# LogicTronixInc/Event-Camera-Clustering-and-Optical-Flow-Estimation

Hardware: AMD Instinct MI355X
Metric: Mevents/s (downsample+cluster+corner) (higher is better)
Workload: dtype u16xy/i64t (int), fp32 k-means; 1 GPU; e2e hash-downsample(8192-event windows) -> k-means k=16 (10 iters) on reps -> SAE+FAST arc corners (16384-event slices) -> 15x15 NMS; 346x260 sensor; 20004864 events/GPU/step (BASELINE configs C2-C4); events_per_gpu=20004864, events_total=20004864, preset=c4, reps_per_gpu=7697279, width=346, height=260, k=16, kmeans_iters=10, parallelism=time-window shards x1, launch=eager launches, streams=two streams sharing all CUs

## Files before the change

### event-camera-clustering-and-optical-flow-estimation_amd/csrc/corner_flags.hip

```cpp
#include "corner_common.hpp"

namespace {

#ifndef ECC_FLAG_THREADS
#define ECC_FLAG_THREADS 256
#endif
constexpr int kFlagThreads = ECC_FLAG_THREADS;
#ifndef ECC_FLAG_QUADS
#define ECC_FLAG_QUADS 8
#endif
constexpr int kFlagQuads = ECC_FLAG_QUADS;
constexpr int kFlagBatch = kFlagQuads * kFlagThreads;

template <bool kStaged>
__device__ __forceinline__ uint32_t corner_bit(uint32_t v, const CornerGeom &g, const uint32_t *sb,
                                               const uint32_t *__restrict__ rg, int j) {
    const int x = ecc::xy_x(v), y = ecc::xy_y(v);
    if (x >= g.W || y >= g.H) return 0u;
    const int tile = (y / kTile) * g.tiles_x + x / kTile;
    const int lp = (y % kTile) * kTile + x % kTile;
    if (kStaged) return (sb[tile * kSegWords + (lp >> 5)] >> (lp & 31)) & 1u;
    return (rg[(int64_t)tile * kSegWords + (lp >> 5)] >> (lp & 31)) & 1u;
}

template <bool kStaged, bool kCand>
__global__ void __launch_bounds__(kFlagThreads)
flags_event_kernel(const uint32_t *__restrict__ xy, CornerGeom g, const uint32_t *__restrict__ res,
                   const int32_t *__restrict__ first_border, uint8_t *__restrict__ flags, uint32_t *__restrict__ cand,
                   int32_t *__restrict__ n_cand) {
    extern __shared__ uint32_t sb[];
    __shared__ int ctot[kFlagQuads][kFlagThreads / 64];
    const int64_t s = blockIdx.x;
    const int64_t lo = s * g.S;
    const int len = (int)((lo + g.S < g.n ? lo + g.S : g.n) - lo);
    const int j = (int)(s % kGroup);
    const int live_end = s < g.first_detect ? 0 : (g.border_mode == 1 ? min(len, max(first_border[s], 0)) : len);
    const uint32_t *rg = res + s * g.seg_stride;
    const bool vec = ((lo + (int64_t)(reinterpret_cast<uintptr_t>(flags) & 3)) & 3) == 0;
    const int n4 = vec ? len / 4 : 0;
    const int lane = threadIdx.x & 63, wave = threadIdx.x >> 6;
    const __amdgpu_buffer_rsrc_t vq = ecc::buffer_view(xy + lo, (uint32_t)n4 * 16u);
    uint4 pre[kFlagQuads];
    auto load_batch = [&](int q0) {
#pragma unroll
        for (int u = 0; u < kFlagQuads; ++u)
            pre[u] = ecc::buffer_load_u128(vq, threadIdx.x * 16u, (uint32_t)(q0 + u * kFlagThreads) * 16u);
        __builtin_amdgcn_sched_barrier(0);
    };
    load_batch(0);
    if (kStaged && live_end > 0) {
        const int total = g.n_tiles * kSegWords;
        const __amdgpu_buffer_rsrc_t vr = ecc::buffer_view(rg, (uint32_t)total * 4u);
        for (int k0 = 0; k0 < total; k0 += 16 * kFlagThreads) {
            uint4 a[4];
#pragma unroll
            for (int b = 0; b < 4; ++b) a[b] = ecc::buffer_load_u128(vr, (uint32_t)(k0 + 4 * (b * kFlagThreads + (int)threadIdx.x)) * 4u);
            __builtin_amdgcn_sched_barrier(0);
#pragma unroll
            for (int b = 0; b < 4; ++b) {
                const int k = k0 + 4 * (b * kFlagThreads + (int)threadIdx.x);
                if (k + 3 < total) {
                    *reinterpret_cast<uint4 *>(sb + k) = a[b];
                } else {
                    if (k < total) sb[k] = a[b].x;
                    if (k + 1 < total) sb[k + 1] = a[b].y;
                    if (k + 2 < total) sb[k + 2] = a[b].z;
                }
            }
        }
    }
    __syncthreads();
    auto quad_flags = [&](int i, const uint4 v) {
        return corner_bit<kStaged>(v.x, g, sb, rg, j) | (i + 1 < live_end ? corner_bit<kStaged>(v.y, g, sb, rg, j) << 8 : 0u) |
               (i + 2 < live_end ? corner_bit<kStaged>(v.z, g, sb, rg, j) << 16 : 0u) |
               (i + 3 < live_end ? corner_bit<kStaged>(v.w, g, sb, rg, j) << 24 : 0u);
    };
    const uint64_t lt = lane == 0 ? 0ull : (~0ull >> (64 - lane));
    int base = 0;
    uint32_t *dst = cand + lo;
    for (int q0 = 0; q0 < n4; q0 += kFlagBatch) {
        if (q0 > 0) load_batch(q0);
        uint32_t f[kFlagQuads];
        int pfx[kFlagQuads];
#pragma unroll
        for (int u = 0; u < kFlagQuads; ++u) {
            const int q = q0 + u * kFlagThreads + (int)threadIdx.x;
            const int i = 4 * q;
            f[u] = (q < n4 && i < live_end) ? quad_flags(i, pre[u]) : 0u;
            if (q < n4) *reinterpret_cast<uint32_t *>(flags + lo + i) = f[u];
            if constexpr (kCand) {
                const int c = __popc(f[u]);
                const uint64_t b0 = __ballot(c & 1), b1 = __ballot(c & 2), b2 = __ballot(c & 4);
                pfx[u] = __popcll(b0 & lt) + 2 * __popcll(b1 & lt) + 4 * __popcll(b2 & lt);
                if (lane == 0) ctot[u][wave] = __popcll(b0) + 2 * __popcll(b1) + 4 * __popcll(b2);
            }
        }
        if constexpr (kCand) {
            __syncthreads();
#pragma unroll
            for (int u = 0; u < kFlagQuads; ++u) {
                int off = base + pfx[u];
#pragma unroll
                for (int w = 0; w < kFlagThreads / 64; ++w) {
                    const int tw = ctot[u][w];
                    off += w < wave ? tw : 0;
                    base += tw;
                }
                if (f[u]) {
                    if (f[u] & 0x1u) dst[off++] = pre[u].x;
                    if (f[u] & 0x100u) dst[off++] = pre[u].y;
                    if (f[u] & 0x10000u) dst[off++] = pre[u].z;
                    if (f[u] & 0x1000000u) dst[off++] = pre[u].w;
                }
            }
            __syncthreads();
        }
    }
    if constexpr (kCand) {
        if (threadIdx.x == 0) {
            for (int i = 4 * n4; i < len; ++i) {
                const uint32_t v = xy[lo + i];
                const uint32_t fb = i < live_end ? corner_bit<kStaged>(v, g, sb, rg, j) : 0u;
                flags[lo + i] = (uint8_t)fb;
                if (fb) dst[base++] = v;
            }
            n_cand[s] = base;
        }
    } else {
        for (int i = 4 * n4 + threadIdx.x; i < len; i += kFlagThreads)
            flags[lo + i] = (uint8_t)(i < live_end ? corner_bit<kStaged>(xy[lo + i], g, sb, rg, j) : 0u);
    }
}

}

int ecc::corner::launch_flags(ecc_ctx *ctx, hipStream_t s, const uint32_t *xy, const CornerGeom &g, const GroupImages &gi,
                              const int32_t *first_border, uint8_t *corner_flags, uint32_t *cand, int32_t *n_cand) {
    ECC_TIMED(ctx, s, "flags_kernel");
    constexpr size_t kLdsMax = kFlagDynLdsMax;
    const size_t lds = (size_t)g.n_tiles * kSegWords * sizeof(uint32_t);
    if (lds <= kLdsMax) {
        const auto fn = cand ? &flags_event_kernel<true, true> : &flags_event_kernel<true, false>;
        if (lds > 65536)
            if (int rc = ecc::allow_dynamic_lds(ctx, fn, (int)kLdsMax, "flags LDS")) return rc;
        if (cand)
            hipLaunchKernelGGL((flags_event_kernel<true, true>), dim3((unsigned)g.n_slices), dim3(kFlagThreads), lds, s,
                               xy, g, (const uint32_t *)gi.res, first_border, corner_flags, cand, n_cand);
        else
            hipLaunchKernelGGL((flags_event_kernel<true, false>), dim3((unsigned)g.n_slices), dim3(kFlagThreads), lds,
                               s, xy, g, (const uint32_t *)gi.res, first_border, corner_flags, nullptr, nullptr);
    } else {
        if (cand) return ECC_ERR_INVALID;
        hipLaunchKernelGGL((flags_event_kernel<false, false>), dim3((unsigned)g.n_slices), dim3(kFlagThreads), 0, s,
                           xy, g, (const uint32_t *)gi.res, first_border, corner_flags, nullptr, nullptr);
    }
    return ECC_OK;
}
```

### event-camera-clustering-and-optical-flow-estimation_amd/csrc/downsample.hip

```cpp
#include "ecc_internal.hpp"

namespace {

constexpr int kThreads = 512;
constexpr int kMaxWindow = 16384;
constexpr int kBuckets = 8192;
constexpr uint32_t kEmpty = 0x7fffffffu;
constexpr uint32_t kRepeatBit = 0x80000000u;

template <bool kQuads>
__device__ inline void load4(const uint32_t *__restrict__ xy, int64_t g, int64_t n, uint32_t (&v)[4]) {
    if constexpr (kQuads) {
        const int64_t n4 = n >> 2, qi = g >> 2;
        const uint4 q = reinterpret_cast<const uint4 *>(xy)[qi < n4 ? qi : n4 - 1];
        v[0] = q.x; v[1] = q.y; v[2] = q.z; v[3] = q.w;
    } else {
#pragma unroll
        for (int k = 0; k < 4; ++k) v[k] = xy[g + k < n ? g + k : n - 1];
    }
}

template <int NT, int MAXC, bool kQuads>
__global__ void __launch_bounds__(NT)
downsample_hash_kernel(const uint32_t *__restrict__ xy, int64_t n, int window, int n_chunks,
                       int x_max, int y_max, int mult_x, int mult_y,
                       uint32_t *__restrict__ rep_xy, uint32_t *__restrict__ rep_idx,
                       int32_t *__restrict__ win_unique, int32_t *__restrict__ win_repeated) {
    __shared__ __attribute__((aligned(16))) uint32_t table[kBuckets];
    constexpr int kWaves = NT / 64, kChunk = NT * 4;
    __shared__ int wave_tot[MAXC][kWaves];
    __shared__ int red[kWaves];

    const int tid = threadIdx.x;
    const int wave = tid >> 6;
    const int lane = tid & 63;
    const int64_t w = blockIdx.x;
    const int64_t wbase = w * (int64_t)window;
    const int64_t wend = (wbase + window < n) ? wbase + window : n;

    {
        uint4 *t4 = reinterpret_cast<uint4 *>(table);
        const uint4 e = make_uint4(kEmpty, kEmpty, kEmpty, kEmpty);
        for (int i = tid; i < kBuckets / 4; i += NT) t4[i] = e;
    }

    uint32_t v[MAXC][4];
#pragma unroll
    for (int c = 0; c < MAXC; ++c) {
        if (c < n_chunks) {
            load4<kQuads>(xy, wbase + (int64_t)c * kChunk + 4 * tid, n, v[c]);
        }
    }
    __syncthreads();

    auto bucket = [&](int c, int k) -> uint32_t {
        const int li = c * kChunk + 4 * tid + k;
        const int x = ecc::xy_x(v[c][k]), y = ecc::xy_y(v[c][k]);
        const bool ok = (wbase + li < wend) && x <= x_max && y <= y_max;
        return ok ? (uint32_t)((x * mult_x + y * mult_y) & (kBuckets - 1)) : 0xffffffffu;
    };

#pragma unroll
    for (int c = 0; c < MAXC; ++c) {
        if (c < n_chunks) {
#pragma unroll
            for (int k = 0; k < 4; ++k) {
                const uint32_t h = bucket(c, k);
                if (h != 0xffffffffu) atomicMin(&table[h], (uint32_t)(c * kChunk + 4 * tid + k));
            }
        }
    }
    __syncthreads();

    uint32_t repmask[MAXC];
    int rp = 0;
#pragma unroll
    for (int c = 0; c < MAXC; ++c) {
        repmask[c] = 0;
        if (c < n_chunks) {
#pragma unroll
            for (int k = 0; k < 4; ++k) {
                const uint32_t h = bucket(c, k);
                if (h != 0xffffffffu) {
                    const int li = c * kChunk + 4 * tid + k;
                    const uint32_t first = table[h] & kEmpty;
                    if (first == (uint32_t)li) repmask[c] |= 1u << k;
                    else rp += (atomicOr(&table[h], kRepeatBit) & kRepeatBit) ? 0 : 1;
                }
            }
        }
    }

    int lane_prefix[MAXC];
    const uint64_t lt = (lane == 0) ? 0ull : (~0ull >> (64 - lane));
#pragma unroll
    for (int c = 0; c < MAXC; ++c) {
        lane_prefix[c] = 0;
        if (c < n_chunks) {
            const int r = __popc(repmask[c]);
            const uint64_t b0 = __ballot(r & 1), b1 = __ballot(r & 2), b2 = __ballot(r & 4);
            lane_prefix[c] = __popcll(b0 & lt) + 2 * __popcll(b1 & lt) + 4 * __popcll(b2 & lt);
            if (lane == 0) wave_tot[c][wave] = __popcll(b0) + 2 * __popcll(b1) + 4 * __popcll(b2);
        }
    }
    __syncthreads();

    rp = ecc::wave_sum_i32(rp);
    if (lane == 0) red[wave] = rp;

    int base = 0;
#pragma unroll
    for (int c = 0; c < MAXC; ++c) {
        if (c < n_chunks) {
            int off = base + lane_prefix[c];
            for (int ww = 0; ww < kWaves; ++ww) {
                const int t = wave_tot[c][ww];
                if (ww < wave) off += t;
                base += t;
            }
#pragma unroll
            for (int k = 0; k < 4; ++k) {
                if (repmask[c] & (1u << k)) {
                    const int li = c * kChunk + 4 * tid + k;
                    if (rep_xy) rep_xy[wbase + off] = v[c][k];
                    if (rep_idx) rep_idx[wbase + off] = (uint32_t)(wbase + li);
                    ++off;
                }
            }
        }
    }
    __syncthreads();
    if (tid == 0) {
        int r = 0;
        for (int ww = 0; ww < kWaves; ++ww) r += red[ww];
        if (win_unique) win_unique[w] = base;
        if (win_repeated) win_repeated[w] = r;
    }
}

}

ECC_API void ecc_hash_cfg_default(ecc_hash_cfg *cfg) {
    if (!cfg) return;
    cfg->window = 8192;
    cfg->x_max = 1280;
    cfg->y_max = 720;
    cfg->mult_x = 1619;
    cfg->mult_y = 31;
    cfg->n_buckets = 8192;
}

ECC_API int ecc_downsample_hash(ecc_ctx *ctx, const uint32_t *xy, int64_t n,
                                const ecc_hash_cfg *cfg, uint32_t *rep_xy, uint32_t *rep_idx,
                                int32_t *win_unique, int32_t *win_repeated, ecc_stream_t stream) {
    if (!ctx || !cfg || n < 0 || (n > 0 && !xy)) return ECC_ERR_INVALID;
    if (cfg->window < 1 || cfg->window > kMaxWindow) return ECC_ERR_INVALID;
    if (cfg->n_buckets != kBuckets) return ECC_ERR_INVALID;
    if (cfg->x_max < 0 || cfg->y_max < 0 || cfg->mult_x < 0 || cfg->mult_y < 0) return ECC_ERR_INVALID;
    if ((int64_t)65535 * cfg->mult_x + (int64_t)65535 * cfg->mult_y > INT32_MAX) return ECC_ERR_INVALID;
    if (n == 0) return ECC_OK;
    const int64_t n_win = (n + cfg->window - 1) / cfg->window;
    if (n_win > INT32_MAX) return ECC_ERR_INVALID;
    const int n_chunks = (cfg->window + 4 * kThreads - 1) / (4 * kThreads);
    ECC_CHECK_HIP(ctx, hipSetDevice(ctx->device), "hipSetDevice");
    const bool quads = (cfg->window & 3) == 0 && (n & 3) == 0 && (reinterpret_cast<uintptr_t>(xy) & 15) == 0;
    auto kern = quads ? (n_chunks <= 4 ? downsample_hash_kernel<kThreads, 4, true> : downsample_hash_kernel<kThreads, 8, true>)
                      : (n_chunks <= 4 ? downsample_hash_kernel<kThreads, 4, false> : downsample_hash_kernel<kThreads, 8, false>);
    {
        ECC_TIMED(ctx, ecc::as_stream(stream), "downsample_hash_kernel");
        hipLaunchKernelGGL(kern, dim3((unsigned)n_win), dim3(kThreads), 0, ecc::as_stream(stream), xy,
                           n, cfg->window, n_chunks, cfg->x_max, cfg->y_max, cfg->mult_x, cfg->mult_y,
                           rep_xy, rep_idx, win_unique, win_repeated);
    }
    ECC_CHECK_LAUNCH(ctx, "downsample_hash_kernel");
    return ECC_OK;
}
```

Baseline: 43200 Mevents/s.

## Batch branchless corner-flag decode and restructure hash downsample into batched LDS probes

The corner flag kernel now decodes tile and bit positions with mul24 reciprocal division and clamped addresses, and issues grouped LDS reads before combining bits. Branches are replaced by masks, and flags are written through buffer stores. The hash downsample kernel precomputes byte offsets with per-lane sentinel slots so atomics run unconditionally. It also batches table probes and atomicOr calls, fixes MAXC at 4 (using 1024 threads for large windows), sets launch bounds for occupancy and specializes the output writes. These changes aim to cut ALU work, divergence and LDS latency, at the cost of relying on clamped addresses and more complex, harder-to-maintain code.

```diff
diff --git a/event-camera-clustering-and-optical-flow-estimation_amd/csrc/corner_flags.hip b/event-camera-clustering-and-optical-flow-estimation_amd/csrc/corner_flags.hip
--- a/event-camera-clustering-and-optical-flow-estimation_amd/csrc/corner_flags.hip
+++ b/event-camera-clustering-and-optical-flow-estimation_amd/csrc/corner_flags.hip
@@ -1,4 +1,5 @@
 #include "corner_common.hpp"
+#include "flag_decode.hpp"
 
 namespace {
 
@@ -12,15 +13,29 @@
 constexpr int kFlagQuads = ECC_FLAG_QUADS;
 constexpr int kFlagBatch = kFlagQuads * kFlagThreads;
 
+#ifndef ECC_FLAG_GROUP
+#define ECC_FLAG_GROUP 4
+#endif
+constexpr int kFlagGroup = ECC_FLAG_GROUP;
+static_assert(kFlagQuads % kFlagGroup == 0, "a batch is whole read groups");
+static_assert(kFlagTile == (uint32_t)kTile && kFlagSegWords == (uint32_t)kSegWords, "flag_decode.hpp's tile");
+
 template <bool kStaged>
-__device__ __forceinline__ uint32_t corner_bit(uint32_t v, const CornerGeom &g, const uint32_t *sb,
-                                               const uint32_t *__restrict__ rg, int j) {
-    const int x = ecc::xy_x(v), y = ecc::xy_y(v);
-    if (x >= g.W || y >= g.H) return 0u;
-    const int tile = (y / kTile) * g.tiles_x + x / kTile;
-    const int lp = (y % kTile) * kTile + x % kTile;
-    if (kStaged) return (sb[tile * kSegWords + (lp >> 5)] >> (lp & 31)) & 1u;
-    return (rg[(int64_t)tile * kSegWords + (lp >> 5)] >> (lp & 31)) & 1u;
+__device__ __forceinline__ uint32_t seg_word(uint32_t w, const uint32_t *sb, const uint32_t *__restrict__ rg) {
+    return kStaged ? sb[w] : rg[w];
+}
+
+template <bool kStaged>
+__device__ __forceinline__ uint32_t corner_bit(uint32_t v, const CornerGeom &g, uint32_t last_word, const uint32_t *sb,
+                                               const uint32_t *__restrict__ rg) {
+    const uint32_t x = (uint32_t)ecc::xy_x(v), y = (uint32_t)ecc::xy_y(v);
+    const FlagSlot sl = flag_slot(x, y, (uint32_t)g.tiles_x, last_word);
+    return (seg_word<kStaged>(sl.word, sb, rg) >> sl.bit) & flag_on_sensor(x, y, (uint32_t)g.W, (uint32_t)g.H);
+}
+
+__device__ __forceinline__ uint32_t first_bytes(int r) {
+    const int rc = min(max(r, 0), 4);
+    return rc >= 4 ? 0x01010101u : (0x01010101u & ((1u << (8 * (rc & 3))) - 1u));
 }
 
 template <bool kStaged, bool kCand>
@@ -33,7 +48,7 @@
     const int64_t s = blockIdx.x;
     const int64_t lo = s * g.S;
     const int len = (int)((lo + g.S < g.n ? lo + g.S : g.n) - lo);
-    const int j = (int)(s % kGroup);
+    const uint32_t last_word = (uint32_t)(g.n_tiles * kSegWords - 1);
     const int live_end = s < g.first_detect ? 0 : (g.border_mode == 1 ? min(len, max(first_border[s], 0)) : len);
     const uint32_t *rg = res + s * g.seg_stride;
     const bool vec = ((lo + (int64_t)(reinterpret_cast<uintptr_t>(flags) & 3)) & 3) == 0;
@@ -70,11 +85,8 @@
         }
     }
     __syncthreads();
-    auto quad_flags = [&](int i, const uint4 v) {
-        return corner_bit<kStaged>(v.x, g, sb, rg, j) | (i + 1 < live_end ? corner_bit<kStaged>(v.y, g, sb, rg, j) << 8 : 0u) |
-               (i + 2 < live_end ? corner_bit<kStaged>(v.z, g, sb, rg, j) << 16 : 0u) |
-               (i + 3 < live_end ? corner_bit<kStaged>(v.w, g, sb, rg, j) << 24 : 0u);
-    };
+    const int live_q = min(live_end, 4 * n4);
+    const __amdgpu_buffer_rsrc_t vf = ecc::buffer_view(flags + lo, (uint32_t)n4 * 4u);
     const uint64_t lt = lane == 0 ? 0ull : (~0ull >> (64 - lane));
     int base = 0;
     uint32_t *dst = cand + lo;
@@ -83,11 +95,33 @@
         uint32_t f[kFlagQuads];
         int pfx[kFlagQuads];
 #pragma unroll
+        for (int u0 = 0; u0 < kFlagQuads; u0 += kFlagGroup) {
+            uint32_t wd[kFlagGroup][4], sh[kFlagGroup], ok[kFlagGroup];
+#pragma unroll
+            for (int u = 0; u < kFlagGroup; ++u) {
+                const uint32_t ev[4] = {pre[u0 + u].x, pre[u0 + u].y, pre[u0 + u].z, pre[u0 + u].w};
+                sh[u] = ok[u] = 0u;
+#pragma unroll
+                for (int k = 0; k < 4; ++k) {
+                    const uint32_t x = (uint32_t)ecc::xy_x(ev[k]), y = (uint32_t)ecc::xy_y(ev[k]);
+                    const FlagSlot sl = flag_slot(x, y, (uint32_t)g.tiles_x, last_word);
+                    wd[u][k] = seg_word<kStaged>(sl.word, sb, rg);
+                    sh[u] |= sl.bit << (8 * k);
+                    ok[u] |= flag_on_sensor(x, y, (uint32_t)g.W, (uint32_t)g.H) << (8 * k);
+                }
+            }
+#pragma unroll
+            for (int u = 0; u < kFlagGroup; ++u) {
+                const int i = 4 * (q0 + (u0 + u) * kFlagThreads + (int)threadIdx.x);
+                uint32_t bits = 0u;
+#pragma unroll
+                for (int k = 0; k < 4; ++k) bits |= ((wd[u][k] >> ((sh[u] >> (8 * k)) & 31u)) & 1u) << (8 * k);
+                f[u0 + u] = bits & ok[u] & first_bytes(live_q - i);
+                ecc::buffer_store_u32(f[u0 + u], vf, threadIdx.x * 4u, (uint32_t)(q0 + (u0 + u) * kFlagThreads) * 4u);
+            }
+        }
+#pragma unroll
         for (int u = 0; u < kFlagQuads; ++u) {
-            const int q = q0 + u * kFlagThreads + (int)threadIdx.x;
-            const int i = 4 * q;
-            f[u] = (q < n4 && i < live_end) ? quad_flags(i, pre[u]) : 0u;
-            if (q < n4) *reinterpret_cast<uint32_t *>(flags + lo + i) = f[u];
             if constexpr (kCand) {
                 const int c = __popc(f[u]);
                 const uint64_t b0 = __ballot(c & 1), b1 = __ballot(c & 2), b2 = __ballot(c & 4);
@@ -120,7 +154,7 @@
         if (threadIdx.x == 0) {
             for (int i = 4 * n4; i < len; ++i) {
                 const uint32_t v = xy[lo + i];
-                const uint32_t fb = i < live_end ? corner_bit<kStaged>(v, g, sb, rg, j) : 0u;
+                const uint32_t fb = corner_bit<kStaged>(v, g, last_word, sb, rg) & (i < live_end ? 1u : 0u);
                 flags[lo + i] = (uint8_t)fb;
                 if (fb) dst[base++] = v;
             }
@@ -128,7 +162,7 @@
         }
     } else {
         for (int i = 4 * n4 + threadIdx.x; i < len; i += kFlagThreads)
-            flags[lo + i] = (uint8_t)(i < live_end ? corner_bit<kStaged>(xy[lo + i], g, sb, rg, j) : 0u);
+            flags[lo + i] = (uint8_t)(corner_bit<kStaged>(xy[lo + i], g, last_word, sb, rg) & (i < live_end ? 1u : 0u));
     }
 }
 
diff --git a/event-camera-clustering-and-optical-flow-estimation_amd/csrc/downsample.hip b/event-camera-clustering-and-optical-flow-estimation_amd/csrc/downsample.hip
--- a/event-camera-clustering-and-optical-flow-estimation_amd/csrc/downsample.hip
+++ b/event-camera-clustering-and-optical-flow-estimation_amd/csrc/downsample.hip
@@ -3,8 +3,11 @@
 namespace {
 
 constexpr int kThreads = 512;
+constexpr int kMaxChunks = 4;
+constexpr int kProbe = 16;
 constexpr int kMaxWindow = 16384;
 constexpr int kBuckets = 8192;
+constexpr int kSent = 32;
 constexpr uint32_t kEmpty = 0x7fffffffu;
 constexpr uint32_t kRepeatBit = 0x80000000u;
 
@@ -21,12 +24,12 @@
 }
 
 template <int NT, int MAXC, bool kQuads>
-__global__ void __launch_bounds__(NT)
+__global__ void __launch_bounds__(NT, 8)
 downsample_hash_kernel(const uint32_t *__restrict__ xy, int64_t n, int window, int n_chunks,
                        int x_max, int y_max, int mult_x, int mult_y,
                        uint32_t *__restrict__ rep_xy, uint32_t *__restrict__ rep_idx,
                        int32_t *__restrict__ win_unique, int32_t *__restrict__ win_repeated) {
-    __shared__ __attribute__((aligned(16))) uint32_t table[kBuckets];
+    __shared__ __attribute__((aligned(16))) uint32_t table[kBuckets + kSent];
     constexpr int kWaves = NT / 64, kChunk = NT * 4;
     __shared__ int wave_tot[MAXC][kWaves];
     __shared__ int red[kWaves];
@@ -37,6 +40,7 @@
     const int64_t w = blockIdx.x;
     const int64_t wbase = w * (int64_t)window;
     const int64_t wend = (wbase + window < n) ? wbase + window : n;
+    const int wlen = (int)(wend - wbase);
 
     {
         uint4 *t4 = reinterpret_cast<uint4 *>(table);
@@ -53,43 +57,66 @@
     }
     __syncthreads();
 
-    auto bucket = [&](int c, int k) -> uint32_t {
-        const int li = c * kChunk + 4 * tid + k;
-        const int x = ecc::xy_x(v[c][k]), y = ecc::xy_y(v[c][k]);
-        const bool ok = (wbase + li < wend) && x <= x_max && y <= y_max;
-        return ok ? (uint32_t)((x * mult_x + y * mult_y) & (kBuckets - 1)) : 0xffffffffu;
-    };
-
+    static_assert(MAXC == kMaxChunks, "a lane holds 16 event slots, one representative bit each");
+    constexpr uint32_t kTableBytes = kBuckets * 4u;
+    uint32_t hs[MAXC * 4];
+    uint32_t valid = 0u;
+    const uint32_t sent = kTableBytes + 4u * (uint32_t)(tid & (kSent - 1));
+    const uint32_t mx = (uint32_t)mult_x, my = (uint32_t)mult_y;
 #pragma unroll
     for (int c = 0; c < MAXC; ++c) {
         if (c < n_chunks) {
 #pragma unroll
             for (int k = 0; k < 4; ++k) {
-                const uint32_t h = bucket(c, k);
-                if (h != 0xffffffffu) atomicMin(&table[h], (uint32_t)(c * kChunk + 4 * tid + k));
+                const int li = c * kChunk + 4 * tid + k;
+                const uint32_t x = (uint32_t)ecc::xy_x(v[c][k]), y = (uint32_t)ecc::xy_y(v[c][k]);
+                const bool ok = li < wlen && x <= (uint32_t)x_max && y <= (uint32_t)y_max;
+                uint32_t py, hb;
+                asm("v_mul_u32_u24 %0, %1, %2" : "=v"(py) : "s"(my), "v"(y));
+                asm("v_mad_u32_u24 %0, %1, %2, %3" : "=v"(hb) : "v"(x), "s"(mx), "v"(py));
+                hs[c * 4 + k] = ok ? (hb & (kBuckets - 1)) * 4u : sent;
+                valid |= (ok ? 1u : 0u) << (c * 4 + k);
             }
-        }
-    }
-    __syncthreads();
-
-    uint32_t repmask[MAXC];
-    int rp = 0;
-#pragma unroll
-    for (int c = 0; c < MAXC; ++c) {
-        repmask[c] = 0;
-        if (c < n_chunks) {
-#pragma unroll
-            for (int k = 0; k < 4; ++k) {
-                const uint32_t h = bucket(c, k);
-                if (h != 0xffffffffu) {
-                    const int li = c * kChunk + 4 * tid + k;
-                    const uint32_t first = table[h] & kEmpty;
-                    if (first == (uint32_t)li) repmask[c] |= 1u << k;
-                    else rp += (atomicOr(&table[h], kRepeatBit) & kRepeatBit) ? 0 : 1;
-                }
-            }
-        }
-    }
+        } else {
+#pragma unroll
+            for (int k = 0; k < 4; ++k) hs[c * 4 + k] = sent;
+        }
+    }
+    __builtin_amdgcn_sched_barrier(0);
+    auto slot = [&](int e) { return reinterpret_cast<uint32_t *>(reinterpret_cast<char *>(table) + hs[e]); };
+    uint32_t li0 = 4u * (uint32_t)tid;
+    asm("" : "+v"(li0));
+    auto local_index = [&](int e) { return (uint32_t)((e / 4) * kChunk + e % 4) + li0; };
+
+#pragma unroll
+    for (int e = 0; e < 4 * MAXC; ++e) {
+        if (e % 4 == 0) __builtin_amdgcn_sched_barrier(0);
+        atomicMin(slot(e), local_index(e));
+    }
+    __syncthreads();
+
+    asm("" : "+v"(li0));
+    uint32_t firsts = 0u;
+    uint32_t fresh = 0u;
+#pragma unroll
+    for (int e0 = 0; e0 < 4 * MAXC; e0 += kProbe) {
+        uint32_t w[kProbe];
+        __builtin_amdgcn_sched_barrier(0);
+#pragma unroll
+        for (int e = 0; e < kProbe; ++e) w[e] = *slot(e0 + e) & kEmpty;
+        __builtin_amdgcn_sched_barrier(0);
+#pragma unroll
+        for (int e = 0; e < kProbe; ++e) {
+            const bool first = w[e] == local_index(e0 + e);
+            firsts |= (first ? 1u : 0u) << (e0 + e);
+            w[e] = atomicOr(slot(e0 + e), first ? 0u : kRepeatBit);
+        }
+        __builtin_amdgcn_sched_barrier(0);
+#pragma unroll
+        for (int e = 0; e < kProbe; ++e) fresh |= (~w[e] >> 31) << (e0 + e);
+    }
+    const uint32_t reps = valid & firsts;
+    int rp = __popc(valid & ~firsts & fresh);
 
     int lane_prefix[MAXC];
     const uint64_t lt = (lane == 0) ? 0ull : (~0ull >> (64 - lane));
@@ -97,7 +124,7 @@
     for (int c = 0; c < MAXC; ++c) {
         lane_prefix[c] = 0;
         if (c < n_chunks) {
-            const int r = __popc(repmask[c]);
+            const int r = __popc((reps >> (4 * c)) & 15u);
             const uint64_t b0 = __ballot(r & 1), b1 = __ballot(r & 2), b2 = __ballot(r & 4);
             lane_prefix[c] = __popcll(b0 & lt) + 2 * __popcll(b1 & lt) + 4 * __popcll(b2 & lt);
             if (lane == 0) wave_tot[c][wave] = __popcll(b0) + 2 * __popcll(b1) + 4 * __popcll(b2);
@@ -109,26 +136,33 @@
     if (lane == 0) red[wave] = rp;
 
     int base = 0;
-#pragma unroll
-    for (int c = 0; c < MAXC; ++c) {
-        if (c < n_chunks) {
-            int off = base + lane_prefix[c];
-            for (int ww = 0; ww < kWaves; ++ww) {
-                const int t = wave_tot[c][ww];
-                if (ww < wave) off += t;
-                base += t;
-            }
-#pragma unroll
-            for (int k = 0; k < 4; ++k) {
-                if (repmask[c] & (1u << k)) {
-                    const int li = c * kChunk + 4 * tid + k;
-                    if (rep_xy) rep_xy[wbase + off] = v[c][k];
-                    if (rep_idx) rep_idx[wbase + off] = (uint32_t)(wbase + li);
-                    ++off;
+    asm("" : "+v"(li0));
+    auto write_out = [&](auto has_xy, auto has_idx) {
+#pragma unroll
+        for (int c = 0; c < MAXC; ++c) {
+            if (c < n_chunks) {
+                int off = base + lane_prefix[c];
+                for (int ww = 0; ww < kWaves; ++ww) {
+                    const int t = wave_tot[c][ww];
+                    if (ww < wave) off += t;
+                    base += t;
+                }
+#pragma unroll
+                for (int k = 0; k < 4; ++k) {
+                    if (reps & (1u << (4 * c + k))) {
+                        const int li = (int)local_index(4 * c + k);
+                        if constexpr (has_xy.value) rep_xy[wbase + off] = v[c][k];
+                        if constexpr (has_idx.value) rep_idx[wbase + off] = (uint32_t)(wbase + li);
+                        ++off;
+                    }
                 }
             }
         }
-    }
+    };
+    if (rep_xy && rep_idx) write_out(std::true_type{}, std::true_type{});
+    else if (rep_xy) write_out(std::true_type{}, std::false_type{});
+    else if (rep_idx) write_out(std::false_type{}, std::true_type{});
+    else write_out(std::false_type{}, std::false_type{});
     __syncthreads();
     if (tid == 0) {
         int r = 0;
@@ -161,14 +195,15 @@
     if (n == 0) return ECC_OK;
     const int64_t n_win = (n + cfg->window - 1) / cfg->window;
     if (n_win > INT32_MAX) return ECC_ERR_INVALID;
-    const int n_chunks = (cfg->window + 4 * kThreads - 1) / (4 * kThreads);
+    const int nt = cfg->window > 4 * kMaxChunks * kThreads ? 2 * kThreads : kThreads;
+    const int n_chunks = (cfg->window + 4 * nt - 1) / (4 * nt);
     ECC_CHECK_HIP(ctx, hipSetDevice(ctx->device), "hipSetDevice");
     const bool quads = (cfg->window & 3) == 0 && (n & 3) == 0 && (reinterpret_cast<uintptr_t>(xy) & 15) == 0;
-    auto kern = quads ? (n_chunks <= 4 ? downsample_hash_kernel<kThreads, 4, true> : downsample_hash_kernel<kThreads, 8, true>)
-                      : (n_chunks <= 4 ? downsample_hash_kernel<kThreads, 4, false> : downsample_hash_kernel<kThreads, 8, false>);
+    auto kern = quads ? (nt == kThreads ? downsample_hash_kernel<kThreads, kMaxChunks, true> : downsample_hash_kernel<2 * kThreads, kMaxChunks, true>)
+                      : (nt == kThreads ? downsample_hash_kernel<kThreads, kMaxChunks, false> : downsample_hash_kernel<2 * kThreads, kMaxChunks, false>);
     {
         ECC_TIMED(ctx, ecc::as_stream(stream), "downsample_hash_kernel");
-        hipLaunchKernelGGL(kern, dim3((unsigned)n_win), dim3(kThreads), 0, ecc::as_stream(stream), xy,
+        hipLaunchKernelGGL(kern, dim3((unsigned)n_win), dim3(nt), 0, ecc::as_stream(stream), xy,
                            n, cfg->window, n_chunks, cfg->x_max, cfg->y_max, cfg->mult_x, cfg->mult_y,
                            rep_xy, rep_idx, win_unique, win_repeated);
     }
diff --git a/event-camera-clustering-and-optical-flow-estimation_amd/csrc/flag_decode.hpp b/event-camera-clustering-and-optical-flow-estimation_amd/csrc/flag_decode.hpp
--- /dev/null
+++ b/event-camera-clustering-and-optical-flow-estimation_amd/csrc/flag_decode.hpp
@@ -0,0 +1,35 @@
+#pragma once
+#include <cstdint>
+
+#include "corner_decode.hpp"
+
+#if defined(__HIP_DEVICE_COMPILE__)
+#define ECC_UMUL24(a, b) __umul24((a), (b))
+#define ECC_DECODE_OPAQUE(v) asm("" : "+v"(v))
+#else
+#define ECC_UMUL24(a, b) ((uint32_t)(((a) & 0xffffffu) * ((b) & 0xffffffu)))
+#define ECC_DECODE_OPAQUE(v) ((void)0)
+#endif
+
+constexpr uint32_t kFlagTile = 14;
+constexpr uint32_t kFlagSegWords = 7;
+
+ECC_DECODE_HD uint32_t flag_div14(uint32_t v) { return ECC_UMUL24(v >> 1, 37450u) >> 18; }
+
+struct FlagSlot {
+    uint32_t word;
+    uint32_t bit;
+};
+
+ECC_DECODE_HD FlagSlot flag_slot(uint32_t x, uint32_t y, uint32_t tiles_x, uint32_t last_word) {
+    const uint32_t tx = flag_div14(x), ty = flag_div14(y);
+    const uint32_t lp = (ECC_UMUL24(y, kFlagTile) + x) - (ECC_UMUL24(ty, kFlagTile * kFlagTile) + ECC_UMUL24(tx, kFlagTile));
+    uint32_t col = ECC_UMUL24(tx, kFlagSegWords) + (lp >> 5);
+    ECC_DECODE_OPAQUE(col);
+    const uint32_t w = ECC_UMUL24(ty, (tiles_x & 0x1fffu) * kFlagSegWords) + col;
+    return FlagSlot{w < last_word ? w : last_word, lp & 31u};
+}
+
+ECC_DECODE_HD uint32_t flag_on_sensor(uint32_t x, uint32_t y, uint32_t W, uint32_t H) {
+    return (x < W && y < H) ? 1u : 0u;
+}
```

Result: faster. 43970 Mevents/s (median of 6 runs) (+1.8%).
